# PeterFWS/Structure-PLP-SLAM

Hardware: AMD Instinct MI355X
Metric: frames/sec ORB+LSD extract+match, 640x480 TUM-RGBD, 1/2/4/8 GPU (higher is better)
Workload: dtype u8

## Files before the change

structure-plp-slam_amd/csrc/blur_tile.hpp:

```cpp
#pragma once
#include <hip/hip_runtime.h>
#include "plp_barrier.hpp"
#include <stdint.h>

namespace plp {

constexpr int kBlurTW = 128, kBlurTH = 32, kBlurPad = 8;
constexpr int kBlurRS = kBlurTH / 8;

__device__ __forceinline__ int blur_reflect101(int p, int len) {
    if (len == 1) return 0;
    p = p < 0 ? -p : p;
    p = p >= len ? 2 * (len - 1) - p : p;
    if (__builtin_expect(p < 0 || p >= len, 0))
        while (p < 0 || p >= len) p = p < 0 ? -p : 2 * (len - 1) - p;
    return p;
}

template <int R>
struct BlurTileLds {
    static constexpr int IW = kBlurTW + 2 * kBlurPad;
    static constexpr int IH = kBlurTH + 2 * R;
    static constexpr int NPR = IH / 2;
    uint8_t in[IH * IW];
    uint32_t hs2[NPR * kBlurTW];
};

typedef unsigned short blur_us2 __attribute__((ext_vector_type(2)));
__device__ __forceinline__ uint32_t blur_dot2(uint32_t a, uint32_t b, uint32_t c) {
    return __builtin_amdgcn_udot2(__builtin_bit_cast(blur_us2, a), __builtin_bit_cast(blur_us2, b), c, false);
}

template <int R, class Emit>
__device__ __forceinline__ void blur_tile_compute(BlurTileLds<R>& S, const int* __restrict__ taps, Emit emit) {
    constexpr int K = 2 * R + 1, IW = BlurTileLds<R>::IW, NPR = BlurTileLds<R>::NPR;
    const int tid = threadIdx.x;
    constexpr int RU = (R + 3) / 4 * 4;
    constexpr int OFF = RU - R;
    constexpr int ND = (OFF + 3 + K + 3) / 4;
    uint32_t tp[4][(K + 3 + 3) / 4];
#pragma unroll
    for (int e = 0; e < 4; ++e)
#pragma unroll
        for (int m = 0; m < (K + 3 + 3) / 4; ++m) {
            tp[e][m] = 0;
#pragma unroll
            for (int k = 0; k < 4; ++k) {
                const int t = 4 * m + k - e;
                if (t >= 0 && t < K) tp[e][m] |= (uint32_t)taps[t] << (8 * k);
            }
        }
    for (int i = tid; i < NPR * (kBlurTW / 4); i += 256) {
        const int p = i >> 5, c4 = (i & 31) * 4;
        uint32_t a[2][4];
#pragma unroll
        for (int rr = 0; rr < 2; ++rr) {
            const uint32_t* q = reinterpret_cast<const uint32_t*>(&S.in[(2 * p + rr) * IW + kBlurPad - RU + c4]);
            uint32_t d[ND];
#pragma unroll
            for (int k = 0; k < ND; ++k) d[k] = q[k];
#pragma unroll
            for (int o = 0; o < 4; ++o) {
                constexpr int dummy = 0; (void)dummy;
                const int s = OFF + o, q0 = s >> 2, e = s & 3;
                uint32_t acc = 0;
#pragma unroll
                for (int m = 0; m < (e + K + 3) / 4; ++m) acc = __builtin_amdgcn_udot4(d[q0 + m], tp[e][m], acc, false);
                a[rr][o] = acc;
            }
        }
        uint4 v;
        v.x = a[0][0] | (a[1][0] << 16); v.y = a[0][1] | (a[1][1] << 16); v.z = a[0][2] | (a[1][2] << 16); v.w = a[0][3] | (a[1][3] << 16);
        *reinterpret_cast<uint4*>(&S.hs2[p * kBlurTW + c4]) = v;
    }
    wg_barrier();
    const int cg = tid & 31, strip = tid >> 5;
    const int c4 = cg * 4, r0 = strip * kBlurRS;
    constexpr int NP = K / 2 + 1;
    uint32_t te[NP], to[NP];
#pragma unroll
    for (int j = 0; j < NP; ++j) {
        te[j] = (uint32_t)taps[2 * j] | (2 * j + 1 < K ? (uint32_t)taps[2 * j + 1] << 16 : 0u);
        to[j] = (j > 0 ? (uint32_t)taps[2 * j - 1] : 0u) | ((uint32_t)taps[2 * j] << 16);
    }
    uint4 wp[NP + 1];
#pragma unroll
    for (int j = 0; j <= NP; ++j) wp[j] = *reinterpret_cast<const uint4*>(&S.hs2[(r0 / 2 + j) * kBlurTW + c4]);
    uint32_t rows[kBlurRS];
#pragma unroll
    for (int rr = 0; rr < kBlurRS; ++rr) {
        uint32_t a0 = 32768u, a1 = 32768u, a2 = 32768u, a3 = 32768u;
#pragma unroll
        for (int j = 0; j < NP; ++j) {
            const uint32_t t = (rr & 1) ? to[j] : te[j];
            const uint4 v = wp[rr / 2 + j];
            a0 = blur_dot2(v.x, t, a0); a1 = blur_dot2(v.y, t, a1); a2 = blur_dot2(v.z, t, a2); a3 = blur_dot2(v.w, t, a3);
        }
        rows[rr] = __builtin_amdgcn_perm(a1, a0, 0x0c0c0602u) | __builtin_amdgcn_perm(a3, a2, 0x06020c0cu);
    }
    emit(r0, c4, rows);
}

struct BlurJob { const uint8_t* src; uint8_t* dst; int src_pitch, dst_pitch, w, h, tx0, ty0; };

template <int R> struct BlurPrefetch {
    static constexpr int IW = BlurTileLds<R>::IW, IH = BlurTileLds<R>::IH, DW = IW / 4;
    static constexpr int NPRE = (IH * DW + 255) / 256, NPATCH = (IH * 8 + 255) / 256;
    uint32_t pre[NPRE], patch[NPATCH];
};
template <int R> struct BlurSlot {
    static constexpr int DW = BlurTileLds<R>::IW / 4, QR = 256 / DW, QD = 256 % DW;
    static_assert((BlurPrefetch<R>::NPRE - 1) * QD + DW - 1 < 2 * DW, "a thread's dword index wraps at most once per step");
    int r0, d0;
    __device__ __forceinline__ BlurSlot() { const int tid = threadIdx.x; r0 = tid / DW; d0 = tid - r0 * DW; }
    __device__ __forceinline__ void at(int q, int& r, int& d) const { d = d0 + QD * q; r = r0 + QR * q; if (d >= DW) { d -= DW; ++r; } }
};
template <int R> __device__ __forceinline__ void blur_prefetch(BlurPrefetch<R>& F, const BlurJob& J) {
    constexpr int IW = BlurTileLds<R>::IW, IH = BlurTileLds<R>::IH, DW = IW / 4;
    const int tid = threadIdx.x;
    const BlurSlot<R> slot;
    const bool rows_inside = J.ty0 >= R && J.ty0 + kBlurTH + R <= J.h;
#pragma unroll
    for (int q = 0; q < BlurPrefetch<R>::NPRE; ++q) {
        int r, d;
        slot.at(q, r, d);
        const int x = J.tx0 - kBlurPad + 4 * d;
        int y = J.ty0 + r - R;
        if (!rows_inside) y = blur_reflect101(y, J.h);
        F.pre[q] = 0u;
        if (tid + 256 * q < IH * DW && x >= 0 && x + 3 < J.w) F.pre[q] = *reinterpret_cast<const uint32_t*>(J.src + (uint32_t)(__mul24(y, J.src_pitch) + x));
    }
    const int dr0 = (J.w - 3 - (J.tx0 - kBlurPad) + 3) >> 2;
    if (J.tx0 <= 0 || dr0 < DW) {
// ... 93 lines not shown
```

structure-plp-slam_amd/csrc/orb_context.hip:

```cpp
#include <hip/hip_runtime.h>

#include <algorithm>
#include <cstdio>
#include <cstring>
#include <mutex>
#include <string>
#include <vector>

#include "blur_tile.hpp"
#include "orb_device.hpp"
#include "xcd_map.hpp"
#include "plp_common.hpp"
#include "quadtree_model.hpp"

namespace plp {
void launch_quadtree(hipStream_t st, const LevelDev* d_lv, int n_levels, int n_cells_total, const uint32_t* cell_cand,
                     const int32_t* cell_count, int32_t* sel, int32_t* sel_count, int total_sel_cap, uint32_t* qt_scratch,
                     size_t qt_scratch_frame_stride, int32_t* status, int B, int max_quota);
size_t quadtree_scratch_bytes_per_frame(const LevelDev* h_lv, int n_levels);
}

using namespace plp;

struct plp_orb {
    HostPinned pin;
    plp_orb_params p{};
    std::vector<float> rects;
    int device = 0;
    hipStream_t stream = nullptr;
    OrbScaleTables st;
    OrbGeometry geo;
    std::vector<LevelDev> h_lv;
    int total_blur_tiles = 0;
    DevBuf d_lv, d_cells, d_rs;
    ResizeDev rs{};
    int capB = 0;
    DevBuf pyr, blur, l0copy, cell_cand, cell_count, sel, sel_count, status, qt_scratch, d_mask;
    size_t l0copy_frame_stride = 0, qt_frame_stride = 0;
    int max_quota = 0;
    DevBuf s_kps, s_desc, s_counts;
    DevBuf stereo_corr, stereo_stage;
    int s_cap = 0;
    bool mask_is_initialized = false;
    std::vector<uint8_t> rect_mask;
    int rect_mask_rows = 0, rect_mask_cols = 0;
    bool rect_mask_uploaded = false;
    DevBuf d_rect_mask;
    int last_B = 0;
    OrbPlanes last_planes{};
    hipStream_t last_stream = nullptr;
    bool profiling = false;
    hipEvent_t ev[8] = {};
    double stage_ms[7] = {0, 0, 0, 0, 0, 0, 0};
    long stage_batches = 0;
    std::mutex mu;
};

namespace {

plp_status validate(const plp_orb_params* p) {
    if (!p) return set_error(PLP_ERR_INVALID_ARG, "params is NULL");
    if (p->num_levels == 0 || p->num_levels > (uint32_t)kMaxLevels) return set_error(PLP_ERR_INVALID_ARG, "num_levels must be in [1,16]");
    if (!(p->scale_factor > 1.0f)) return set_error(PLP_ERR_INVALID_ARG, "scale_factor must be > 1");
    if (p->n_mask_rects < 0 || (p->n_mask_rects > 0 && !p->mask_rects)) return set_error(PLP_ERR_INVALID_ARG, "mask_rects");
    for (int i = 0; i < p->n_mask_rects; ++i) {
        const float* v = p->mask_rects + 4 * i;
        if (v[0] >= v[1]) return set_error(PLP_ERR_INVALID_ARG, "x_max must be greater than x_min");
        if (v[2] >= v[3]) return set_error(PLP_ERR_INVALID_ARG, "y_max must be greater than x_min");
    }
    return PLP_OK;
}

void reinitialize(plp_orb* c) {
    c->st = make_scale_tables(c->p.max_num_keypts, c->p.scale_factor, c->p.num_levels);
    c->geo = OrbGeometry{};
}

plp_status build_geometry_impl(plp_orb* c, int rows, int cols);

plp_status build_geometry(plp_orb* c, int rows, int cols) {
    if (c->geo.rows == rows && c->geo.cols == cols && c->geo.n_levels == (int)c->p.num_levels) return PLP_OK;
    const plp_status s = build_geometry_impl(c, rows, cols);
    if (s != PLP_OK) { c->geo = OrbGeometry{}; c->h_lv.clear(); c->capB = 0; }
    return s;
}

plp_status build_geometry_impl(plp_orb* c, int rows, int cols) {
    const int nl = (int)c->p.num_levels;
    {
        OrbGeometry g = make_geometry(rows, cols, c->st, nl);
        for (int l = 0; l < nl; ++l)
            if (g.lv[l].w <= 2 * kOrbBorder + 6 || g.lv[l].h <= 2 * kOrbBorder + 6)
                return set_error(PLP_ERR_INVALID_ARG, "image too small for the requested pyramid (level narrower than 45 px)");
        if (cols - 2 * kOrbBorder > 4095 || rows - 2 * kOrbBorder > 4095)
            return set_error(PLP_ERR_UNSUPPORTED, "images larger than 4133 px are not supported (12-bit candidate packing)");
        c->geo = std::move(g);
    }
    c->h_lv.assign(nl, LevelDev{});
    c->total_blur_tiles = 0;
    size_t qt_off = 0;
    int max_cells = 0;
    for (int l = 0; l < nl; ++l) {
        const LevelGeom& G = c->geo.lv[l];
        LevelDev& L = c->h_lv[l];
        L.w = G.w; L.h = G.h; L.pitch = G.pitch; L.off = G.off;
        L.blur_tiles = ((G.w + 127) / 128) * ((G.h + plp::kBlurTH - 1) / plp::kBlurTH);
        L.blur_tiles_x_magic = plp::plp_div_magic((uint32_t)((G.w + 127) / 128), (uint64_t)L.blur_tiles);
        c->total_blur_tiles += L.blur_tiles;
        L.scale = c->st.sf[l];
        L.sel_base = G.sel_base; L.sel_cap = G.sel_cap;
        L.cell_base = G.cell_base; L.n_cells = G.n_cell_rows * G.n_cell_cols;
        L.quota = (int)c->st.quota[l];
        c->max_quota = l == 0 ? L.quota : std::max(c->max_quota, L.quota);
        L.n_init_x = G.n_init_x; L.delta_x = G.delta_x; L.delta_y = G.delta_y;
        L.qt_cap = std::min(std::max(L.n_cells, 1) * kCellCap, 65535);
        L.qt_off = qt_off;
        qt_off += (size_t)L.qt_cap * 20;
        const int extent = (int)std::ceil(std::max(G.delta_x, G.delta_y)) + 1;
        int t1 = 0;
        while ((1 << t1) < extent) ++t1;
        const int d_eff = std::min(t1 + 2, kQtDepth);
        const int n_init = G.n_init_x * G.n_init_y;
        int nb = 0;
        while ((1 << nb) < n_init) ++nb;
        L.sort_lo = 2 * (kQtDepth - d_eff);
        L.sort_hi = 2 * kQtDepth + nb;
        if (L.n_cells > 2048 || 3 * L.quota + 8 > kQtMaxNodesLdsSmallBlock || n_init > 32)
            return set_error(PLP_ERR_UNSUPPORTED, "frame/keypoint budget exceeds the quadtree kernel limits (quota per level <= 2010, 2048 cells per level, 32 initial nodes)");
        max_cells = std::max(max_cells, L.n_cells);
    }
    if (3 * c->max_quota + 8 > kQtMaxNodesLds && max_cells > 1024)
        return set_error(PLP_ERR_UNSUPPORTED, "frame/keypoint budget exceeds the quadtree kernel limits (a quota above 1960 per level needs levels of at most 1024 cells)");
    PLP_HIP(c->d_lv.upload(c->h_lv.data(), sizeof(LevelDev) * nl, c->stream));
    PLP_HIP(c->d_cells.upload(c->geo.cells.data(), sizeof(CellDesc) * c->geo.cells.size(), c->stream));
    const ResizeTables& R = c->geo.rs;
    const size_t nc = R.xofs0.size(), nr = R.yofs0.size();
    std::vector<int16_t> blob;
    blob.reserve(4 * nc + 4 * nr + 8);
    auto push = [&](const std::vector<int16_t>& v) { size_t o = blob.size(); blob.insert(blob.end(), v.begin(), v.end()); return o; };
    const size_t o0 = push(R.xofs0), o1 = push(R.xofs1), o2 = push(R.a0), o3 = push(R.a1);
    const size_t o4 = push(R.yofs0), o5 = push(R.yofs1), o6 = push(R.b0), o7 = push(R.b1);
    if (blob.empty()) blob.push_back(0);
    PLP_HIP(c->d_rs.upload(blob.data(), blob.size() * 2, c->stream));
    const int16_t* base = (const int16_t*)c->d_rs.p;
    c->rs.xofs0 = base + o0; c->rs.xofs1 = base + o1; c->rs.a0 = base + o2; c->rs.a1 = base + o3;
    c->rs.yofs0 = base + o4; c->rs.yofs1 = base + o5; c->rs.b0 = base + o6; c->rs.b1 = base + o7;
    for (int l = 0; l < nl; ++l) { c->rs.col_base[l] = R.col_base[l]; c->rs.row_base[l] = R.row_base[l]; }
    c->capB = 0;
    PLP_HIP(hipStreamSynchronize(c->stream));
    return PLP_OK;
}

plp_status ensure_capacity(plp_orb* c, int B) {
    if (B <= c->capB) return PLP_OK;
    const OrbGeometry& g = c->geo;
    const size_t n_cells = g.cells.size();
    c->l0copy_frame_stride = ((size_t)g.lv[0].pitch * g.rows + 255) / 256 * 256;
    c->qt_frame_stride = quadtree_scratch_bytes_per_frame(c->h_lv.data(), g.n_levels);
    PLP_HIP(c->pyr.reserve(g.frame_plane_bytes * B));
    PLP_HIP(c->blur.reserve(g.frame_plane_bytes * B));
    PLP_HIP(c->l0copy.reserve(c->l0copy_frame_stride * B));
    PLP_HIP(c->cell_cand.reserve(sizeof(uint32_t) * kCellCap * n_cells * B));
    PLP_HIP(c->cell_count.reserve(sizeof(int32_t) * n_cells * B));
    PLP_HIP(c->sel.reserve(sizeof(int32_t) * g.total_sel_cap * B));
    PLP_HIP(c->sel_count.reserve(sizeof(int32_t) * kMaxLevels * B));
    PLP_HIP(c->status.reserve(sizeof(int32_t) * 4));
    PLP_HIP(c->qt_scratch.reserve(c->qt_frame_stride * B));
// ... 25 lines not shown

    const bool prof = c->profiling;
    static const bool trace = getenv("PLP_TRACE") != nullptr;
    auto mark = [&](int i) {
        if (prof) (void)hipEventRecord(c->ev[i], st);
        if (trace) { const hipError_t e = hipStreamSynchronize(st); fprintf(stderr, "plp_orb: stage boundary %d reached (%dx%d, B=%d)%s\n", i, cols, rows, B, e == hipSuccess ? "" : " ERROR"); fflush(stderr); }
    };
    mark(0);
    OrbPlanes pl{};
    pl.pyr = (uint8_t*)c->pyr.p; pl.pyr_frame_stride = g.frame_plane_bytes;
    const bool aligned = ((uintptr_t)d_imgs % 4 == 0) && (step % 4 == 0) && (frame_stride % 4 == 0);
    if (aligned) { pl.l0 = d_imgs; pl.l0_frame_stride = frame_stride; pl.l0_pitch = (int)step; }
    else {
        for (int f = 0; f < B; ++f)
            PLP_HIP(hipMemcpy2DAsync((uint8_t*)c->l0copy.p + f * c->l0copy_frame_stride, g.lv[0].pitch, d_imgs + f * frame_stride, step,
                                     cols, rows, hipMemcpyDeviceToDevice, st));
        pl.l0 = (const uint8_t*)c->l0copy.p; pl.l0_frame_stride = c->l0copy_frame_stride; pl.l0_pitch = g.lv[0].pitch;
    }
    build_rect_mask(c, rows, cols);
    if (!d_mask && !c->rect_mask.empty()) {
        if (c->rect_mask_rows != rows || c->rect_mask_cols != cols)
            return set_error(PLP_ERR_INVALID_ARG, "rectangle mask was built for a different frame size");
        if (!c->rect_mask_uploaded) {
            PLP_HIP(c->d_rect_mask.upload(c->rect_mask.data(), c->rect_mask.size(), st));
            c->rect_mask_uploaded = true;
        }
        d_mask = (const uint8_t*)c->d_rect_mask.p; mask_step = cols; mask_frame_stride = 0;
    }

    PLP_HIP(hipMemsetAsync(c->status.p, 0, 16, st));
    mark(1);
    for (int l = 1; l < nl; ++l) launch_resize(st, pl, c->h_lv.data(), l, B, c->rs);
    mark(2);
    launch_fast(st, pl, (const CellDesc*)c->d_cells.p, (int)g.cells.size(), (const LevelDev*)c->d_lv.p, B, (int)c->p.ini_fast_thr,
                (int)c->p.min_fast_thr, d_mask, mask_step, mask_frame_stride, (uint32_t*)c->cell_cand.p, (int32_t*)c->cell_count.p);
    mark(3);
    BlurTaps taps{{18, 34, 48, 56, 48, 34, 18}};
    launch_blur(st, pl, (uint8_t*)c->blur.p, g.frame_plane_bytes, (const LevelDev*)c->d_lv.p, nl, c->total_blur_tiles, B, taps, c->h_lv.data());
    mark(4);
    launch_quadtree(st, (const LevelDev*)c->d_lv.p, nl, (int)g.cells.size(), (const uint32_t*)c->cell_cand.p,
                    (const int32_t*)c->cell_count.p, (int32_t*)c->sel.p, (int32_t*)c->sel_count.p, g.total_sel_cap,
                    (uint32_t*)c->qt_scratch.p, c->qt_frame_stride, (int32_t*)c->status.p, B, c->max_quota);
    mark(5);
    UMax um;
    for (int v = 0; v <= kHalfPatch; ++v) um.v[v] = c->st.u_max[v];
    launch_orient_rbrief(st, pl, (const uint8_t*)c->blur.p, g.frame_plane_bytes, (const LevelDev*)c->d_lv.p, nl, (const int32_t*)c->sel.p,
                         (const int32_t*)c->sel_count.p, g.total_sel_cap, um, d_kps, d_desc, cap, d_counts, (int32_t*)c->status.p, B);
    PLP_HIP(hipGetLastError());
    if (trace) { const hipError_t e = hipStreamSynchronize(st); fprintf(stderr, "plp_orb: batch done%s\n", e == hipSuccess ? "" : " ERROR"); fflush(stderr); }
    if (prof) {
        mark(6);
        PLP_HIP(hipEventSynchronize(c->ev[6]));
        for (int i = 0; i < 6; ++i) { float ms = 0; PLP_HIP(hipEventElapsedTime(&ms, c->ev[i], c->ev[i + 1])); c->stage_ms[i] += ms; }
        float tot = 0; PLP_HIP(hipEventElapsedTime(&tot, c->ev[0], c->ev[6])); c->stage_ms[6] += tot;
        ++c->stage_batches;
    }
    c->last_B = B; c->last_planes = pl; c->last_stream = st;
    return PLP_OK;
}

}

extern "C" {

void plp_orb_default_params(plp_orb_params* p) {
    if (!p) return;
    p->max_num_keypts = 2000; p->scale_factor = 1.2f; p->num_levels = 8; p->ini_fast_thr = 20; p->min_fast_thr = 7;
    p->mask_rects = nullptr; p->n_mask_rects = 0;
}

plp_status plp_orb_create(const plp_orb_params* params, int device, plp_orb** out) {
// ... 294 lines not shown
```

structure-plp-slam_amd/csrc/orb_device.hpp:

```cpp
#pragma once
#include <hip/hip_runtime.h>
#include <stdint.h>

#include "../../include/plp_front.h"
#include "orb_tables.hpp"

namespace plp {

constexpr int kQtMaxNodesLds = 5888;
constexpr int kQtMaxNodesLdsSmallBlock = 6040;

struct LevelDev {
    int w, h, pitch;
    int blur_tiles;
    uint32_t blur_tiles_x_magic;
    size_t off;
    float scale;
    int sel_base, sel_cap;
    int cell_base, n_cells;
    int quota;
    int n_init_x;
    double delta_x, delta_y;
    size_t qt_off;
    int qt_cap;
    int sort_lo, sort_hi;
};

struct OrbPlanes {
    const uint8_t* l0; size_t l0_frame_stride; int l0_pitch;
    uint8_t* pyr; size_t pyr_frame_stride;
    __host__ __device__ const uint8_t* level_ptr(int frame, int level, const LevelDev& L) const {
        return level == 0 ? l0 + (size_t)frame * l0_frame_stride : pyr + (size_t)frame * pyr_frame_stride + L.off;
    }
    __host__ __device__ int level_pitch(int level, const LevelDev& L) const { return level == 0 ? l0_pitch : L.pitch; }
};

struct BlurTaps { int k[7]; };
struct UMax { int v[kHalfPatch + 1]; };

struct ResizeDev {
    const int16_t *xofs0, *xofs1, *a0, *a1, *yofs0, *yofs1, *b0, *b1;
    int col_base[kMaxLevels], row_base[kMaxLevels];
};

struct StereoArgs {
    const plp_keypoint *kps_l, *kps_r;
    const uint8_t *desc_l, *desc_r;
    const int32_t *cnt_l, *cnt_r;
    int cap;
    float fxb, tb;
    float inv_scale[kMaxLevels];
    float* x_right; float* depth;
    int32_t* corr;
};
void launch_stereo(hipStream_t st, const OrbPlanes& pl_l, const OrbPlanes& pl_r, const LevelDev* d_lv, const StereoArgs& A, int B);

void launch_resize(hipStream_t st, const OrbPlanes& pl, const LevelDev* h_lv, int level, int B, const ResizeDev& rs);
void launch_fast(hipStream_t st, const OrbPlanes& pl, const CellDesc* d_cells, int n_cells, const LevelDev* d_lv, int B,
                 int ini_thr, int min_thr, const uint8_t* d_mask, size_t mask_step, size_t mask_frame_stride,
                 uint32_t* cell_cand, int32_t* cell_count);
void launch_blur(hipStream_t st, const OrbPlanes& pl, uint8_t* blur, size_t blur_frame_stride, const LevelDev* d_lv,
                 int n_levels, int total_tiles, int B, const BlurTaps& taps, const LevelDev* h_lv = nullptr);
void launch_orient_rbrief(hipStream_t st, const OrbPlanes& pl, const uint8_t* blur, size_t blur_frame_stride,
                          const LevelDev* d_lv, int n_levels, const int32_t* sel, const int32_t* sel_count,
                          int total_sel_cap, const UMax& um, plp_keypoint* kps, uint8_t* desc, int cap, int32_t* counts,
                          int32_t* status, int B);

}
```

structure-plp-slam_amd/csrc/orb_kernels.hip:

```cpp
#include <hip/hip_runtime.h>
#include <stdint.h>

#include "blur_tile.hpp"
#include "plp_barrier.hpp"
#include "orb_device.hpp"
#include "plp_common.hpp"
#include "xcd_map.hpp"

namespace plp {

__device__ __forceinline__ int rs_tab(const int16_t* __restrict__ t, int i) { return *reinterpret_cast<const int16_t*>(reinterpret_cast<const char*>(t) + ((uint32_t)i << 1)); }
constexpr int kRsRows = 44, kRsPitch = 96;

__global__ __launch_bounds__(256) __attribute__((amdgpu_waves_per_eu(7, 8))) void k_resize_linear(const uint8_t* __restrict__ src_base, size_t src_frame_stride,
                                                       int src_pitch, int sw, uint8_t* __restrict__ dst_base,
                                                       size_t dst_frame_stride, int dst_pitch, int dw, int dh,
                                                       const int16_t* __restrict__ xofs0, const int16_t* __restrict__ xofs1,
                                                       const int16_t* __restrict__ a0, const int16_t* __restrict__ a1,
                                                       const int16_t* __restrict__ yofs0, const int16_t* __restrict__ yofs1,
                                                       const int16_t* __restrict__ b0, const int16_t* __restrict__ b1) {
    constexpr int ROWS = 8;
    __shared__ __attribute__((aligned(16))) uint8_t tiles[4 * kRsRows * kRsPitch];
    const int lane = threadIdx.x & 63, wv = __builtin_amdgcn_readfirstlane((int)(threadIdx.x >> 6));
    const int strip_x0 = blockIdx.x * 64, strip_y0 = (blockIdx.y * 4 + wv) * 32;
// ... 78 lines not shown
            cached_row = y1;
            *reinterpret_cast<uint32_t*>(dst + (uint32_t)(__mul24(dy, dst_pitch) + dx0)) = packed;
        }
        return;
    }
    for (int r = 0; r < ROWS; ++r) {
        const int dy = dy0 + r;
        if (dy >= dh) break;
        const uint8_t* S0 = src + (size_t)yofs0[dy] * src_pitch;
        const uint8_t* S1 = src + (size_t)yofs1[dy] * src_pitch;
        const int wb0 = b0[dy], wb1 = b1[dy];
        uint32_t packed = 0;
#pragma unroll
        for (int i = 0; i < 4; ++i) {
            const int h0 = S0[x0[i]] * wa0[i] + S0[x1[i]] * wa1[i];
            const int h1 = S1[x0[i]] * wa0[i] + S1[x1[i]] * wa1[i];
            const int v = (((wb0 * (h0 >> 4)) >> 16) + ((wb1 * (h1 >> 4)) >> 16) + 2) >> 2;
            packed |= (uint32_t)(v & 255) << (8 * i);
        }
        *reinterpret_cast<uint32_t*>(dst + (size_t)dy * dst_pitch + dx0) = packed;
    }
}

constexpr int kFastQ1 = 1536, kFastQ2 = 512;
constexpr int kTileW = 76;
constexpr int kScoreW = 68;

__device__ __forceinline__ int min3(int a, int b, int c) { return min(a, min(b, c)); }

__global__ __launch_bounds__(256) __attribute__((amdgpu_waves_per_eu(8, 8))) void k_fast_cells(OrbPlanes pl, const CellDesc* __restrict__ cells,
                                                    const LevelDev* __restrict__ lv, int ini_thr, int min_thr,
                                                    const uint8_t* __restrict__ mask, size_t mask_step,
                                                    size_t mask_frame_stride, uint32_t* __restrict__ cell_cand,
                                                    int32_t* __restrict__ cell_count, int n_cells, uint32_t gx_magic) {
    __shared__ __attribute__((aligned(16))) uint8_t tile[70 * kTileW];
    __shared__ __attribute__((aligned(16))) uint8_t score[66 * kScoreW];
    __shared__ unsigned long long keepbits[64];
    __shared__ uint16_t queue[kFastQ1], queue2[kFastQ2];
    __shared__ unsigned long long bits1[64], bits2[64];
    __shared__ int q_count, q2_count, n_ini, wave_tot[4], run_base;

    unsigned ucell, uframe;
    xcd_frame_major(ucell, uframe, gx_magic);
    const int tid = threadIdx.x, frame = (int)uframe, cell = (int)ucell;
    const CellDesc cd = cells[cell];
    const LevelDev L = lv[cd.level];
    const int out_slot = frame * n_cells + cell;
    const float sf = L.scale;

    const uint8_t* mk = mask ? mask + (size_t)frame * mask_frame_stride : nullptr;
    auto masked = [&](int y, int x) -> bool {
        return mk[(size_t)(int)((float)y * sf) * mask_step + (int)((float)x * sf)] == 0;
    };
    if (mk) {
        const int x0 = cd.min_x, x1 = cd.min_x + cd.w, y0 = cd.min_y, y1 = cd.min_y + cd.h;
        if (masked(y0, x0) || masked(y1, x0) || masked(y0, x1) || masked(y1, x1)) {
            if (tid == 0) cell_count[out_slot] = 0;
            return;
        }
    }

    const uint8_t* img = pl.level_ptr(frame, cd.level, L);
    const int pitch = pl.level_pitch(cd.level, L);
    const int w = cd.w, h = cd.h;
    {
        const int a0 = cd.min_x - 1;
        const int sh = a0 & 3;
        const int ndw = (w + 2 + 3) >> 2;
        const uint8_t* row0 = img + (size_t)cd.min_y * pitch + (a0 - sh);
        const int qr = 256 / ndw, qd = 256 - qr * ndw;
        int r = tid / ndw, c = tid - r * ndw;
        for (int i = tid; i < ndw * h; i += 256, c += qd, r += qr) {
            if (c >= ndw) { c -= ndw; ++r; }
            const uint32_t* g = reinterpret_cast<const uint32_t*>(row0 + (ptrdiff_t)(__mul24(r, pitch) + 4 * c));
            const uint32_t lo = g[0];
            const uint32_t v = sh ? __builtin_amdgcn_alignbyte(g[1], lo, (uint32_t)sh) : lo;
            *reinterpret_cast<uint32_t*>(&tile[r * kTileW + 4 * c]) = v;
        }
    }
    const int tw = w - 6, th = h - 6;
    int thr = ini_thr;
    for (int attempt = 0; attempt < 2; ++attempt) {
        thr = attempt == 0 ? ini_thr : min_thr;
        for (int i = tid; i < 66 * kScoreW / 4; i += 256) reinterpret_cast<uint32_t*>(score)[i] = 0;
        if (tid < 64) { keepbits[tid] = 0ull; bits1[tid] = 0ull; bits2[tid] = 0ull; }
        if (tid == 0) { q_count = 0; q2_count = 0; n_ini = 0; run_base = 0; }
        wg_barrier();
        for (int i = tid; i < 1024; i += 256) {
            const int ty = i >> 4, tx4 = (i & 15) * 4;
            if (tx4 >= tw || ty >= th) continue;
            const uint32_t* rowc = reinterpret_cast<const uint32_t*>(&tile[(ty + 3) * kTileW]) + (tx4 >> 2);
            const uint32_t C = rowc[1], Lw = rowc[0], Rw = rowc[2];
            const uint32_t Lq = __builtin_amdgcn_alignbyte(C, Lw, 1u);
            const uint32_t Rq = __builtin_amdgcn_alignbyte(Rw, C, 3u);
            const uint32_t U = *(reinterpret_cast<const uint32_t*>(&tile[ty * kTileW]) + (tx4 >> 2) + 1);
            const uint32_t D = *(reinterpret_cast<const uint32_t*>(&tile[(ty + 6) * kTileW]) + (tx4 >> 2) + 1);
#pragma unroll
            for (int k = 0; k < 4; ++k) {
                if (tx4 + k >= tw) break;
                const int v = (int)((C >> (8 * k)) & 255u);
                const int hi = v + thr, lo = v - thr;
                const int p0 = (int)((D >> (8 * k)) & 255u), p4 = (int)((Rq >> (8 * k)) & 255u), p8 = (int)((U >> (8 * k)) & 255u),
                          p12 = (int)((Lq >> (8 * k)) & 255u);
                const bool b0 = p0 > hi, b4 = p4 > hi, b8 = p8 > hi, b12 = p12 > hi;
                const bool d0 = p0 < lo, d4 = p4 < lo, d8 = p8 < lo, d12 = p12 < lo;
                if (((b0 | b8) & (b4 | b12)) | ((d0 | d8) & (d4 | d12))) {
                    atomicOr(&bits1[ty], 1ull << (tx4 + k));
                    const int slot = atomicAdd(&q_count, 1);
                    if (slot < kFastQ1) queue[slot] = (uint16_t)((ty << 6) | (tx4 + k));
                }
            }
        }
        wg_barrier();
// ... 117 lines not shown
    wg_barrier();
    int off = 0;
    for (int k = 0; k < wv; ++k) off += wave_tot[k];
    for (int ty = 16 * wv; ty < 16 * wv + 16; ++ty) {
        const unsigned long long m = row_mask(ty);
        if ((m >> lane) & 1ull) {
            const uint32_t v = score[(ty + 1) * kScoreW + lane + 1];
            const uint32_t x = (uint32_t)(lane + 3 + cd.cx * kCellSize), y = (uint32_t)(ty + 3 + cd.cy * kCellSize);
            out[off + __popcll(m & ((1ull << lane) - 1ull))] = x | (y << 12) | (v << 24);
        }
        off += __popcll(m);
    }
    if (tid == 0) run_base = wave_tot[0] + wave_tot[1] + wave_tot[2] + wave_tot[3];
    wg_barrier();
    if (tid == 0) cell_count[out_slot] = run_base;
}

__global__ __launch_bounds__(256) __attribute__((amdgpu_waves_per_eu(8, 8))) void k_blur7(OrbPlanes pl, uint8_t* __restrict__ blur_base, size_t blur_frame_stride,
                                               const LevelDev* __restrict__ lv, int n_levels, BlurTaps taps, uint32_t gx_magic) {
    __shared__ BlurTileLds<3> S;
    unsigned ut, uf;
    xcd_frame_major(ut, uf, gx_magic);
    int t = (int)ut;
    const int frame = (int)uf;
    int level = 0;
    while (level + 1 < n_levels && t >= lv[level].blur_tiles) { t -= lv[level].blur_tiles; ++level; }
    const LevelDev L = lv[level];
    const int tiles_x = (L.w + kBlurTW - 1) / kBlurTW;
    const int trow = (int)plp_div((unsigned)t, (unsigned)tiles_x, L.blur_tiles_x_magic);
    blur_tile<3>(S, pl.level_ptr(frame, level, L), pl.level_pitch(level, L), blur_base + (size_t)frame * blur_frame_stride + L.off, L.pitch,
                 L.w, L.h, (t - trow * tiles_x) * kBlurTW, trow * kBlurTH, taps.k);
}

__device__ __forceinline__ float fast_atan2_deg(float y, float x) {
    const float p1 = 0.9997878412794807f * (float)(180 / 3.14159265358979323846);
    const float p3 = -0.3258083974640975f * (float)(180 / 3.14159265358979323846);
    const float p5 = 0.1555786518463281f * (float)(180 / 3.14159265358979323846);
    const float p7 = -0.04432655554792128f * (float)(180 / 3.14159265358979323846);
    const float eps = (float)2.2204460492503131e-16;
    const float ax = fabsf(x), ay = fabsf(y);
    float a;
    if (ax >= ay) {
        const float c = __fdiv_rn(ay, __fadd_rn(ax, eps));
        const float c2 = __fmul_rn(c, c);
        a = __fmul_rn(__fadd_rn(__fmul_rn(__fadd_rn(__fmul_rn(__fadd_rn(__fmul_rn(p7, c2), p5), c2), p3), c2), p1), c);
    } else {
        const float c = __fdiv_rn(ax, __fadd_rn(ay, eps));
        const float c2 = __fmul_rn(c, c);
        a = __fsub_rn(90.f, __fmul_rn(__fadd_rn(__fmul_rn(__fadd_rn(__fmul_rn(__fadd_rn(__fmul_rn(p7, c2), p5), c2), p3), c2), p1), c));
    }
    if (x < 0) a = __fsub_rn(180.f, a);
    if (y < 0) a = __fsub_rn(360.f, a);
    return a;
}

__device__ __forceinline__ float ref_poly_cos(float v) {
    const float v2 = __fmul_rn(v, v);
    return __fadd_rn(0.99940307f, __fmul_rn(v2, __fadd_rn(-0.49558072f, __fmul_rn(0.03679168f, v2))));
}
__device__ __forceinline__ float ref_cos(float v) {
    const float PI = 3.14159265358979f, PI_2 = PI / 2.0f, TWO_PI = 2.0f * PI, INV_TWO_PI = 1.0f / TWO_PI, THREE_PI_2 = 3.0f * PI_2;
    const float q = __fmul_rn(v, INV_TWO_PI);
    int fl = (int)q;
    fl -= (fl > q);
    v = __fsub_rn(v, __fmul_rn((float)fl, TWO_PI));
    v = (0.0f < v) ? v : -v;
// ... 137 lines not shown
    }
#pragma unroll
    for (int r = 0; r < 16; ++r) bits |= (uint32_t)(ta[r] < tb[r]) << r;
    reinterpret_cast<uint16_t*>(out_desc + ((size_t)frame * cap + out_idx) * 32)[sub] = (uint16_t)bits;
    if (sub == 0) {
        plp_keypoint k;
        const float s = L.scale;
        k.x = level ? __fmul_rn((float)cx, s) : (float)cx;
        k.y = level ? __fmul_rn((float)cy, s) : (float)cy;
        k.size = (float)(unsigned)(__fmul_rn((float)kFastPatch, s));
        k.angle = angle;
        k.response = (float)resp;
        k.octave = level;
        k.class_id = -1;
        out_kps[(size_t)frame * cap + out_idx] = k;
    }
}

void launch_resize(hipStream_t st, const OrbPlanes& pl, const LevelDev* h_lv, int level, int B, const ResizeDev& rs) {
    const LevelDev& S = h_lv[level - 1];
    const LevelDev& D = h_lv[level];
    const uint8_t* src = level - 1 == 0 ? pl.l0 : pl.pyr + S.off;
    const size_t sstride = level - 1 == 0 ? pl.l0_frame_stride : pl.pyr_frame_stride;
    const int spitch = level - 1 == 0 ? pl.l0_pitch : S.pitch;
    dim3 grid((D.w + 63) / 64, (D.h + 127) / 128, B), block(256);
    hipLaunchKernelGGL(k_resize_linear, grid, block, 0, st, src, sstride, spitch, S.w, pl.pyr + D.off, pl.pyr_frame_stride, D.pitch,
                       D.w, D.h, rs.xofs0 + rs.col_base[level], rs.xofs1 + rs.col_base[level], rs.a0 + rs.col_base[level],
                       rs.a1 + rs.col_base[level], rs.yofs0 + rs.row_base[level], rs.yofs1 + rs.row_base[level],
                       rs.b0 + rs.row_base[level], rs.b1 + rs.row_base[level]);
}

void launch_fast(hipStream_t st, const OrbPlanes& pl, const CellDesc* d_cells, int n_cells, const LevelDev* d_lv, int B,
                 int ini_thr, int min_thr, const uint8_t* d_mask, size_t mask_step, size_t mask_frame_stride,
                 uint32_t* cell_cand, int32_t* cell_count) {
    hipLaunchKernelGGL(k_fast_cells, dim3(n_cells, B), dim3(256), 0, st, pl, d_cells, d_lv, ini_thr, min_thr, d_mask, mask_step,
                       mask_frame_stride, cell_cand, cell_count, n_cells, plp_div_magic((uint32_t)n_cells, (uint64_t)n_cells * B));
}

void launch_blur(hipStream_t st, const OrbPlanes& pl, uint8_t* blur, size_t blur_frame_stride, const LevelDev* d_lv,
                 int n_levels, int total_tiles, int B, const BlurTaps& taps, const LevelDev* h_lv) {
    (void)h_lv;
    hipLaunchKernelGGL(k_blur7, dim3(total_tiles, B), dim3(256), 0, st, pl, blur, blur_frame_stride, d_lv, n_levels, taps, plp_div_magic((uint32_t)total_tiles, (uint64_t)total_tiles * B));
}

void launch_orient_rbrief(hipStream_t st, const OrbPlanes& pl, const uint8_t* blur, size_t blur_frame_stride,
                          const LevelDev* d_lv, int n_levels, const int32_t* sel, const int32_t* sel_count,
                          int total_sel_cap, const UMax& um, plp_keypoint* kps, uint8_t* desc, int cap, int32_t* counts,
                          int32_t* status, int B) {
    hipLaunchKernelGGL(k_orient_rbrief, dim3((total_sel_cap + 15) / 16, B), dim3(256), 0, st, pl, blur, blur_frame_stride, d_lv,
                       n_levels, sel, sel_count, total_sel_cap, um, kps, desc, cap, counts, status,
                       plp_div_magic((uint32_t)((total_sel_cap + 15) / 16), (uint64_t)((total_sel_cap + 15) / 16) * B));
}

__global__ __launch_bounds__(256) void k_stereo_match(OrbPlanes pl_l, OrbPlanes pl_r, const LevelDev* __restrict__ lv, StereoArgs A) {
    const int lane = threadIdx.x & 63, b = blockIdx.y;
    const int il = blockIdx.x * 4 + __builtin_amdgcn_readfirstlane((int)(threadIdx.x >> 6));
    const int nl = A.cnt_l ? min(A.cnt_l[b], A.cap) : A.cap, nr = A.cnt_r ? min(A.cnt_r[b], A.cap) : A.cap;
    if (il >= A.cap) return;
    float* xr_out = A.x_right + (size_t)b * A.cap;
    float* dp_out = A.depth + (size_t)b * A.cap;
    int32_t* corr_out = A.corr + (size_t)b * A.cap;
    if (lane == 0) { xr_out[il] = -1.0f; dp_out[il] = -1.0f; corr_out[il] = -1; }
    if (il >= nl) return;
    const plp_keypoint kp = A.kps_l[(size_t)b * A.cap + il];
    const plp_keypoint* kr = A.kps_r + (size_t)b * A.cap;
    const float max_disp = __fdiv_rn(A.fxb, A.tb), min_disp = 0.0f;
    const int row = (int)(unsigned long long)kp.y;
    const float min_x = __fsub_rn(kp.x, max_disp), max_x = __fsub_rn(kp.x, min_disp);
    if (max_x < 0) return;
// ... 106 lines not shown
```

structure-plp-slam_amd/csrc/orb_tables.hpp:

```cpp
#pragma once
#include <algorithm>
#include <cmath>
#include <cstdint>
#include <vector>

namespace plp {

constexpr int kOrbBorder = 19;
constexpr int kFastPatch = 31;
constexpr int kHalfPatch = 15;
constexpr int kCellSize = 64;
constexpr int kCellOverlap = 6;
constexpr int kMaxLevels = 16;
constexpr int kCellCap = 1024;

struct OrbScaleTables {
    std::vector<float> sf, isf, sigma2, isigma2;
    std::vector<uint32_t> quota;
    int u_max[kHalfPatch + 1];
};

inline OrbScaleTables make_scale_tables(uint32_t max_kp, float scale_factor, uint32_t n_levels) {
    OrbScaleTables t;
    t.sf.assign(n_levels, 1.0f); t.isf.assign(n_levels, 1.0f);
// ... 18 lines not shown
    t.quota[n_levels - 1] = (uint32_t)std::max((int)max_kp - (int)used, 0);
    const double r = kHalfPatch;
    const int vmax = (int)std::floor(r * std::sqrt(2.0) / 2 + 1);
    const int vmin = (int)std::ceil(r * std::sqrt(2.0) / 2);
    for (int v = 0; v <= kHalfPatch; ++v) t.u_max[v] = 0;
    for (int v = 0; v <= vmax; ++v) t.u_max[v] = (int)std::round(std::sqrt(r * r - (double)v * v));
    for (int v = kHalfPatch, v0 = 0; v >= vmin; --v) {
        while (t.u_max[v0] == t.u_max[v0 + 1]) ++v0;
        t.u_max[v] = v0;
        ++v0;
    }
    return t;
}

inline int floor_i(float v) { int i = (int)v; return i - (i > v); }
inline short q11(float w) {
    const int i = (int)std::nearbyintf(w * 2048);
    return (short)std::min(std::max(i, -32768), 32767);
}

struct LevelGeom {
    int w = 0, h = 0, pitch = 0;
    size_t off = 0;
    int n_cell_cols = 0, n_cell_rows = 0;
    int cell_base = 0;
    int max_bx = 0, max_by = 0;
    int n_init_x = 1, n_init_y = 1;
    double delta_x = 0, delta_y = 0;
    int sel_cap = 0, sel_base = 0;
};

struct CellDesc {
    int32_t level, min_x, min_y, w;
    int32_t h, cx, cy, pad;
};

struct ResizeTables {
    std::vector<int16_t> xofs0, xofs1, a0, a1;
    std::vector<int16_t> yofs0, yofs1, b0, b1;
    std::vector<int> col_base, row_base;
};

struct OrbGeometry {
    int rows = 0, cols = 0, n_levels = 0;
    std::vector<LevelGeom> lv;
    std::vector<CellDesc> cells;
    size_t frame_plane_bytes = 0;
    int total_sel_cap = 0;
    ResizeTables rs;
};

inline OrbGeometry make_geometry(int rows, int cols, const OrbScaleTables& st, int n_levels) {
    OrbGeometry g;
    g.rows = rows; g.cols = cols; g.n_levels = n_levels;
    g.lv.resize(n_levels);
    size_t off = 0;
    for (int l = 0; l < n_levels; ++l) {
        LevelGeom& L = g.lv[l];
        if (l == 0) { L.w = cols; L.h = rows; }
        else {
            const double scale = st.sf[l];
            L.w = (int)std::round(cols * 1.0 / scale);
            L.h = (int)std::round(rows * 1.0 / scale);
        }
        L.pitch = (L.w + 63) / 64 * 64;
        L.off = off;
        off += ((size_t)L.pitch * L.h + 255) / 256 * 256;
// ... 76 lines not shown
```

Before: 91500.

## Fuse Gaussian blur into FAST cell kernel, blur only uncovered borders separately

The FAST cell kernel already loads each cell's image tile into LDS, so it now also computes the 7-tap Gaussian blur of the cell interior from that tile and writes it out. This avoids a second read of the pyramid by the separate blur pass. A new border kernel blurs only the strips not covered by cell interiors, using wide or tall tiles. The old full blur path stays available through an environment variable. The cost is more LDS pressure and extra work and barriers in the FAST kernel, and the border kernel adds a launch.

```diff
diff --git a/structure-plp-slam_amd/csrc/blur_tile.hpp b/structure-plp-slam_amd/csrc/blur_tile.hpp
--- a/structure-plp-slam_amd/csrc/blur_tile.hpp
+++ b/structure-plp-slam_amd/csrc/blur_tile.hpp
@@ -31,9 +31,10 @@
     return __builtin_amdgcn_udot2(__builtin_bit_cast(blur_us2, a), __builtin_bit_cast(blur_us2, b), c, false);
 }
 
-template <int R, class Emit>
-__device__ __forceinline__ void blur_tile_compute(BlurTileLds<R>& S, const int* __restrict__ taps, Emit emit) {
-    constexpr int K = 2 * R + 1, IW = BlurTileLds<R>::IW, NPR = BlurTileLds<R>::NPR;
+template <int R, int TW, int IP, class Emit>
+__device__ __forceinline__ void blur_block_compute(const uint8_t* in0, uint32_t* hs2, const int* __restrict__ taps, Emit emit) {
+    constexpr int K = 2 * R + 1, CG = TW / 4, TH = 4096 / TW, NPR = TH / 2 + R;
+    static_assert((CG & (CG - 1)) == 0 && CG <= 256 && IP % 4 == 0, "column groups: a power of two");
     const int tid = threadIdx.x;
     constexpr int RU = (R + 3) / 4 * 4;
     constexpr int OFF = RU - R;
@@ -50,12 +51,12 @@
                 if (t >= 0 && t < K) tp[e][m] |= (uint32_t)taps[t] << (8 * k);
             }
         }
-    for (int i = tid; i < NPR * (kBlurTW / 4); i += 256) {
-        const int p = i >> 5, c4 = (i & 31) * 4;
+    for (int i = tid; i < NPR * CG; i += 256) {
+        const int p = (int)((unsigned)i / CG), c4 = (int)((unsigned)i % CG) * 4;
         uint32_t a[2][4];
 #pragma unroll
         for (int rr = 0; rr < 2; ++rr) {
-            const uint32_t* q = reinterpret_cast<const uint32_t*>(&S.in[(2 * p + rr) * IW + kBlurPad - RU + c4]);
+            const uint32_t* q = reinterpret_cast<const uint32_t*>(&in0[(2 * p + rr) * IP + c4]);
             uint32_t d[ND];
 #pragma unroll
             for (int k = 0; k < ND; ++k) d[k] = q[k];
@@ -71,10 +72,10 @@
         }
         uint4 v;
         v.x = a[0][0] | (a[1][0] << 16); v.y = a[0][1] | (a[1][1] << 16); v.z = a[0][2] | (a[1][2] << 16); v.w = a[0][3] | (a[1][3] << 16);
-        *reinterpret_cast<uint4*>(&S.hs2[p * kBlurTW + c4]) = v;
+        *reinterpret_cast<uint4*>(&hs2[p * TW + c4]) = v;
     }
     wg_barrier();
-    const int cg = tid & 31, strip = tid >> 5;
+    const int cg = (int)((unsigned)tid % CG), strip = (int)((unsigned)tid / CG);
     const int c4 = cg * 4, r0 = strip * kBlurRS;
     constexpr int NP = K / 2 + 1;
     uint32_t te[NP], to[NP];
@@ -85,7 +86,7 @@
     }
     uint4 wp[NP + 1];
 #pragma unroll
-    for (int j = 0; j <= NP; ++j) wp[j] = *reinterpret_cast<const uint4*>(&S.hs2[(r0 / 2 + j) * kBlurTW + c4]);
+    for (int j = 0; j <= NP; ++j) wp[j] = *reinterpret_cast<const uint4*>(&hs2[(r0 / 2 + j) * TW + c4]);
     uint32_t rows[kBlurRS];
 #pragma unroll
     for (int rr = 0; rr < kBlurRS; ++rr) {
@@ -99,6 +100,13 @@
         rows[rr] = __builtin_amdgcn_perm(a1, a0, 0x0c0c0602u) | __builtin_amdgcn_perm(a3, a2, 0x06020c0cu);
     }
     emit(r0, c4, rows);
+}
+
+template <int R, class Emit>
+__device__ __forceinline__ void blur_tile_compute(BlurTileLds<R>& S, const int* __restrict__ taps, Emit emit) {
+    constexpr int RU = (R + 3) / 4 * 4;
+    static_assert(4096 / kBlurTW == kBlurTH && BlurTileLds<R>::NPR == kBlurTH / 2 + R, "tile shape");
+    blur_block_compute<R, kBlurTW, BlurTileLds<R>::IW>(&S.in[kBlurPad - RU], S.hs2, taps, emit);
 }
 
 struct BlurJob { const uint8_t* src; uint8_t* dst; int src_pitch, dst_pitch, w, h, tx0, ty0; };
diff --git a/structure-plp-slam_amd/csrc/orb_context.hip b/structure-plp-slam_amd/csrc/orb_context.hip
--- a/structure-plp-slam_amd/csrc/orb_context.hip
+++ b/structure-plp-slam_amd/csrc/orb_context.hip
@@ -32,7 +32,8 @@
     OrbGeometry geo;
     std::vector<LevelDev> h_lv;
     int total_blur_tiles = 0;
-    DevBuf d_lv, d_cells, d_rs;
+    std::vector<BlurStrip> blur_strips;
+    DevBuf d_lv, d_cells, d_rs, d_strips;
     ResizeDev rs{};
     int capB = 0;
     DevBuf pyr, blur, l0copy, cell_cand, cell_count, sel, sel_count, status, qt_scratch, d_mask;
@@ -77,6 +78,40 @@
 }
 
 plp_status build_geometry_impl(plp_orb* c, int rows, int cols);
+
+void build_blur_coverage(std::vector<CellDesc>& cells, const std::vector<LevelDev>& lv, std::vector<BlurStrip>& strips) {
+    strips.clear();
+    auto add = [&](int l, int x0, int x1, int y0, int y1, bool wide) {
+        if (x0 >= x1 || y0 >= y1) return;
+        const int tw = wide ? kBlurTW : 4096 / kBlurTW, th = 4096 / tw;
+        for (int ty = y0; ty < y1; ty += th)
+            for (int tx = x0 & ~3; tx < x1; tx += tw) strips.push_back({l, tx, ty, wide ? 1 : 0, x0, x1, y0, y1});
+    };
+    for (int l = 0; l < (int)lv.size(); ++l) {
+        const LevelDev& L = lv[l];
+        int ix0 = L.w, ix1 = 0, iy0 = L.h, iy1 = 0;
+        long long area = 0;
+        for (int k = L.cell_base; k < L.cell_base + L.n_cells; ++k) {
+            const CellDesc& a = cells[k];
+            ix0 = std::min(ix0, a.min_x + 3); ix1 = std::max(ix1, a.min_x + a.w - 3);
+            iy0 = std::min(iy0, a.min_y + 3); iy1 = std::max(iy1, a.min_y + a.h - 3);
+            area += (long long)(a.w - 6) * (a.h - 6);
+        }
+        bool tiled = L.n_cells > 0 && ix0 >= 3 && iy0 >= 3 && ix1 <= L.w - 3 && iy1 <= L.h - 3 && area == (long long)(ix1 - ix0) * (iy1 - iy0);
+        for (int k = L.cell_base; tiled && k < L.cell_base + L.n_cells; ++k)
+            for (int m = k + 1; tiled && m < L.cell_base + L.n_cells; ++m) {
+                const CellDesc &a = cells[k], &b = cells[m];
+                tiled = a.w <= 6 || b.w <= 6 || a.h <= 6 || b.h <= 6 || a.min_x + a.w - 3 <= b.min_x + 3 || b.min_x + b.w - 3 <= a.min_x + 3 ||
+                        a.min_y + a.h - 3 <= b.min_y + 3 || b.min_y + b.h - 3 <= a.min_y + 3;
+            }
+        for (int k = L.cell_base; k < L.cell_base + L.n_cells; ++k) cells[k].blur = tiled ? 1 : 0;
+        if (!tiled) { add(l, 0, L.w, 0, L.h, true); continue; }
+        add(l, 0, L.w, 0, iy0, true);
+        add(l, 0, L.w, iy1, L.h, true);
+        add(l, 0, ix0, iy0, iy1, false);
+        add(l, ix1, L.w, iy0, iy1, false);
+    }
+}
 
 plp_status build_geometry(plp_orb* c, int rows, int cols) {
     if (c->geo.rows == rows && c->geo.cols == cols && c->geo.n_levels == (int)c->p.num_levels) return PLP_OK;
@@ -131,8 +166,10 @@
     }
     if (3 * c->max_quota + 8 > kQtMaxNodesLds && max_cells > 1024)
         return set_error(PLP_ERR_UNSUPPORTED, "frame/keypoint budget exceeds the quadtree kernel limits (a quota above 1960 per level needs levels of at most 1024 cells)");
+    build_blur_coverage(c->geo.cells, c->h_lv, c->blur_strips);
     PLP_HIP(c->d_lv.upload(c->h_lv.data(), sizeof(LevelDev) * nl, c->stream));
     PLP_HIP(c->d_cells.upload(c->geo.cells.data(), sizeof(CellDesc) * c->geo.cells.size(), c->stream));
+    if (!c->blur_strips.empty()) PLP_HIP(c->d_strips.upload(c->blur_strips.data(), sizeof(BlurStrip) * c->blur_strips.size(), c->stream));
     const ResizeTables& R = c->geo.rs;
     const size_t nc = R.xofs0.size(), nr = R.yofs0.size();
     std::vector<int16_t> blob;
@@ -224,11 +261,17 @@
     mark(1);
     for (int l = 1; l < nl; ++l) launch_resize(st, pl, c->h_lv.data(), l, B, c->rs);
     mark(2);
+    static const bool separate_blur = [] { const char* e = getenv("PLP_ORB_BLUR"); return e && strcmp(e, "separate") == 0; }();
+    const BlurTaps taps{{18, 34, 48, 56, 48, 34, 18}};
     launch_fast(st, pl, (const CellDesc*)c->d_cells.p, (int)g.cells.size(), (const LevelDev*)c->d_lv.p, B, (int)c->p.ini_fast_thr,
-                (int)c->p.min_fast_thr, d_mask, mask_step, mask_frame_stride, (uint32_t*)c->cell_cand.p, (int32_t*)c->cell_count.p);
+                (int)c->p.min_fast_thr, d_mask, mask_step, mask_frame_stride, (uint32_t*)c->cell_cand.p, (int32_t*)c->cell_count.p,
+                separate_blur ? nullptr : (uint8_t*)c->blur.p, g.frame_plane_bytes, taps);
     mark(3);
-    BlurTaps taps{{18, 34, 48, 56, 48, 34, 18}};
-    launch_blur(st, pl, (uint8_t*)c->blur.p, g.frame_plane_bytes, (const LevelDev*)c->d_lv.p, nl, c->total_blur_tiles, B, taps, c->h_lv.data());
+    if (separate_blur)
+        launch_blur(st, pl, (uint8_t*)c->blur.p, g.frame_plane_bytes, (const LevelDev*)c->d_lv.p, nl, c->total_blur_tiles, B, taps, c->h_lv.data());
+    else
+        launch_blur_border(st, pl, (uint8_t*)c->blur.p, g.frame_plane_bytes, (const LevelDev*)c->d_lv.p, (const BlurStrip*)c->d_strips.p,
+                           (int)c->blur_strips.size(), B, taps);
     mark(4);
     launch_quadtree(st, (const LevelDev*)c->d_lv.p, nl, (int)g.cells.size(), (const uint32_t*)c->cell_cand.p,
                     (const int32_t*)c->cell_count.p, (int32_t*)c->sel.p, (int32_t*)c->sel_count.p, g.total_sel_cap,
diff --git a/structure-plp-slam_amd/csrc/orb_device.hpp b/structure-plp-slam_amd/csrc/orb_device.hpp
--- a/structure-plp-slam_amd/csrc/orb_device.hpp
+++ b/structure-plp-slam_amd/csrc/orb_device.hpp
@@ -36,6 +36,8 @@
 };
 
 struct BlurTaps { int k[7]; };
+
+struct BlurStrip { int level, tx0, ty0, wide, x0, x1, y0, y1; };
 struct UMax { int v[kHalfPatch + 1]; };
 
 struct ResizeDev {
@@ -58,7 +60,9 @@
 void launch_resize(hipStream_t st, const OrbPlanes& pl, const LevelDev* h_lv, int level, int B, const ResizeDev& rs);
 void launch_fast(hipStream_t st, const OrbPlanes& pl, const CellDesc* d_cells, int n_cells, const LevelDev* d_lv, int B,
                  int ini_thr, int min_thr, const uint8_t* d_mask, size_t mask_step, size_t mask_frame_stride,
-                 uint32_t* cell_cand, int32_t* cell_count);
+                 uint32_t* cell_cand, int32_t* cell_count, uint8_t* blur, size_t blur_frame_stride, const BlurTaps& taps);
+void launch_blur_border(hipStream_t st, const OrbPlanes& pl, uint8_t* blur, size_t blur_frame_stride, const LevelDev* d_lv,
+                        const BlurStrip* d_strips, int n_strips, int B, const BlurTaps& taps);
 void launch_blur(hipStream_t st, const OrbPlanes& pl, uint8_t* blur, size_t blur_frame_stride, const LevelDev* d_lv,
                  int n_levels, int total_tiles, int B, const BlurTaps& taps, const LevelDev* h_lv = nullptr);
 void launch_orient_rbrief(hipStream_t st, const OrbPlanes& pl, const uint8_t* blur, size_t blur_frame_stride,
diff --git a/structure-plp-slam_amd/csrc/orb_kernels.hip b/structure-plp-slam_amd/csrc/orb_kernels.hip
--- a/structure-plp-slam_amd/csrc/orb_kernels.hip
+++ b/structure-plp-slam_amd/csrc/orb_kernels.hip
@@ -134,12 +134,21 @@
                                                     const LevelDev* __restrict__ lv, int ini_thr, int min_thr,
                                                     const uint8_t* __restrict__ mask, size_t mask_step,
                                                     size_t mask_frame_stride, uint32_t* __restrict__ cell_cand,
-                                                    int32_t* __restrict__ cell_count, int n_cells, uint32_t gx_magic) {
+                                                    int32_t* __restrict__ cell_count, int n_cells, uint32_t gx_magic,
+                                                    uint8_t* __restrict__ blur_base, size_t blur_frame_stride, BlurTaps taps) {
     __shared__ __attribute__((aligned(16))) uint8_t tile[70 * kTileW];
-    __shared__ __attribute__((aligned(16))) uint8_t score[66 * kScoreW];
+    struct FastScratch {
+        uint8_t score[66 * kScoreW];
+        uint16_t queue[kFastQ1], queue2[kFastQ2];
+        unsigned long long bits1[64], bits2[64];
+    };
+    __shared__ __attribute__((aligned(16))) union { FastScratch f; uint32_t hs2[(32 + 3) * 64]; } U;
+    auto& score = U.f.score;
     __shared__ unsigned long long keepbits[64];
-    __shared__ uint16_t queue[kFastQ1], queue2[kFastQ2];
-    __shared__ unsigned long long bits1[64], bits2[64];
+    auto& queue = U.f.queue;
+    auto& queue2 = U.f.queue2;
+    auto& bits1 = U.f.bits1;
+    auto& bits2 = U.f.bits2;
     __shared__ int q_count, q2_count, n_ini, wave_tot[4], run_base;
 
     unsigned ucell, uframe;
@@ -154,11 +163,14 @@
     auto masked = [&](int y, int x) -> bool {
         return mk[(size_t)(int)((float)y * sf) * mask_step + (int)((float)x * sf)] == 0;
     };
+    const bool blur_cell = blur_base != nullptr && cd.blur != 0;
+    bool skipped = false;
     if (mk) {
         const int x0 = cd.min_x, x1 = cd.min_x + cd.w, y0 = cd.min_y, y1 = cd.min_y + cd.h;
         if (masked(y0, x0) || masked(y1, x0) || masked(y0, x1) || masked(y1, x1)) {
             if (tid == 0) cell_count[out_slot] = 0;
-            return;
+            if (!blur_cell) return;
+            skipped = true;
         }
     }
 
@@ -181,6 +193,27 @@
         }
     }
     const int tw = w - 6, th = h - 6;
+    if (blur_cell) {
+        static_assert((kOrbBorder + 3) % 2 == 0 && kCellSize % 4 == 0, "interior columns start 2-byte aligned: 16-bit stores");
+        wg_barrier();
+        uint8_t* dst = blur_base + (size_t)frame * blur_frame_stride + L.off + (size_t)(cd.min_y + 3) * L.pitch + (cd.min_x + 3);
+        blur_block_compute<3, 64, kTileW>(tile, U.hs2, taps.k, [&](int r0, int c4, const uint32_t (&rows)[kBlurRS]) {
+            const int n = min(tw - c4, 4);
+            if (n <= 0) return;
+#pragma unroll
+            for (int rr = 0; rr < kBlurRS; ++rr) {
+                if (r0 + rr >= th) break;
+                uint8_t* p = dst + (uint32_t)__mul24(r0 + rr, L.pitch) + c4;
+                if (n == 4) {
+                    reinterpret_cast<uint16_t*>(p)[0] = (uint16_t)rows[rr];
+                    reinterpret_cast<uint16_t*>(p)[1] = (uint16_t)(rows[rr] >> 16);
+                } else
+                    for (int k = 0; k < n; ++k) p[k] = (uint8_t)(rows[rr] >> (8 * k));
+            }
+        });
+        wg_barrier();
+        if (skipped) return;
+    }
     int thr = ini_thr;
     for (int attempt = 0; attempt < 2; ++attempt) {
         thr = attempt == 0 ? ini_thr : min_thr;
@@ -364,6 +397,78 @@
                  L.w, L.h, (t - trow * tiles_x) * kBlurTW, trow * kBlurTH, taps.k);
 }
 
+struct BorderEmit {
+    uint8_t* dst; int pitch, tx0, ty0, x0, x1, y0, y1;
+    __device__ __forceinline__ void operator()(int r0, int c4, const uint32_t (&rows)[kBlurRS]) const {
+        const int x = tx0 + c4;
+        if (x >= x1 || x + 4 <= x0) return;
+        const bool whole = x >= x0 && x + 4 <= x1;
+#pragma unroll
+        for (int rr = 0; rr < kBlurRS; ++rr) {
+            const int y = ty0 + r0 + rr;
+            if (y < y0 || y >= y1) continue;
+            uint8_t* p = dst + (size_t)y * pitch + x;
+            if (whole) *reinterpret_cast<uint32_t*>(p) = rows[rr];
+            else
+                for (int k = 0; k < 4; ++k)
+                    if (x + k >= x0 && x + k < x1) p[k] = (uint8_t)(rows[rr] >> (8 * k));
+        }
+    }
+};
+
+struct TallLds {
+    static constexpr int TW = 32, TH = 4096 / TW, IW = TW + 8, IH = TH + 6;
+    uint8_t in[IH * IW];
+    __attribute__((aligned(16))) uint32_t hs2[(TH / 2 + 3) * TW];
+};
+
+__device__ __forceinline__ void blur7_tall_tile(TallLds& S, const uint8_t* __restrict__ src, int src_pitch, int w, int h, int tx0, int ty0,
+                                                const int* __restrict__ taps, const BorderEmit& emit) {
+    constexpr int IW = TallLds::IW, IH = TallLds::IH, DW = IW / 4, N = IH * DW, NQ = (N + 255) / 256;
+    const int tid = threadIdx.x;
+    uint32_t v[NQ];
+    const uint8_t* rowp[NQ];
+#pragma unroll
+    for (int q = 0; q < NQ; ++q) {
+        const int i = min(tid + 256 * q, N - 1), r = (int)((unsigned)i / DW), d = i - r * DW;
+        rowp[q] = src + (size_t)blur_reflect101(ty0 - 3 + r, h) * src_pitch;
+        v[q] = *reinterpret_cast<const uint32_t*>(rowp[q] + min(max(tx0 - 4 + 4 * d, 0), w - 4));
+    }
+#pragma unroll
+    for (int q = 0; q < NQ; ++q) {
+        const int i = min(tid + 256 * q, N - 1), r = (int)((unsigned)i / DW), d = i - r * DW;
+        const int x = tx0 - 4 + 4 * d;
+        if (x < 0 || x + 3 >= w) {
+            uint32_t b = 0u;
+#pragma unroll
+            for (int k = 0; k < 4; ++k) b |= (uint32_t)rowp[q][blur_reflect101(x + k, w)] << (8 * k);
+            v[q] = b;
+        }
+    }
+#pragma unroll
+    for (int q = 0; q < NQ; ++q) {
+        const int i = tid + 256 * q, r = (int)((unsigned)i / DW), d = i - r * DW;
+        if (i < N) *reinterpret_cast<uint32_t*>(&S.in[r * IW + 4 * d]) = v[q];
+    }
+    wg_barrier();
+    blur_block_compute<3, TallLds::TW, IW>(S.in, S.hs2, taps, emit);
+}
+
+__global__ __launch_bounds__(256) __attribute__((amdgpu_waves_per_eu(8, 8))) void k_blur7_border(OrbPlanes pl, uint8_t* __restrict__ blur_base, size_t blur_frame_stride,
+                                                      const LevelDev* __restrict__ lv, const BlurStrip* __restrict__ strips, BlurTaps taps, uint32_t gx_magic) {
+    __shared__ __attribute__((aligned(16))) union { BlurTileLds<3> wide; TallLds tall; } S;
+    unsigned ut, uf;
+    xcd_frame_major(ut, uf, gx_magic);
+    const int frame = (int)uf;
+    const BlurStrip J = strips[ut];
+    const LevelDev L = lv[J.level];
+    const uint8_t* src = pl.level_ptr(frame, J.level, L);
+    const int src_pitch = pl.level_pitch(J.level, L);
+    const BorderEmit emit{blur_base + (size_t)frame * blur_frame_stride + L.off, L.pitch, J.tx0, J.ty0, J.x0, J.x1, J.y0, J.y1};
+    if (J.wide) blur_tile_core<3>(S.wide, src, src_pitch, L.w, L.h, J.tx0, J.ty0, taps.k, emit);
+    else blur7_tall_tile(S.tall, src, src_pitch, L.w, L.h, J.tx0, J.ty0, taps.k, emit);
+}
+
 __device__ __forceinline__ float fast_atan2_deg(float y, float x) {
     const float p1 = 0.9997878412794807f * (float)(180 / 3.14159265358979323846);
     const float p3 = -0.3258083974640975f * (float)(180 / 3.14159265358979323846);
@@ -567,9 +672,17 @@
 
 void launch_fast(hipStream_t st, const OrbPlanes& pl, const CellDesc* d_cells, int n_cells, const LevelDev* d_lv, int B,
                  int ini_thr, int min_thr, const uint8_t* d_mask, size_t mask_step, size_t mask_frame_stride,
-                 uint32_t* cell_cand, int32_t* cell_count) {
+                 uint32_t* cell_cand, int32_t* cell_count, uint8_t* blur, size_t blur_frame_stride, const BlurTaps& taps) {
     hipLaunchKernelGGL(k_fast_cells, dim3(n_cells, B), dim3(256), 0, st, pl, d_cells, d_lv, ini_thr, min_thr, d_mask, mask_step,
-                       mask_frame_stride, cell_cand, cell_count, n_cells, plp_div_magic((uint32_t)n_cells, (uint64_t)n_cells * B));
+                       mask_frame_stride, cell_cand, cell_count, n_cells, plp_div_magic((uint32_t)n_cells, (uint64_t)n_cells * B),
+                       blur, blur_frame_stride, taps);
+}
+
+void launch_blur_border(hipStream_t st, const OrbPlanes& pl, uint8_t* blur, size_t blur_frame_stride, const LevelDev* d_lv,
+                        const BlurStrip* d_strips, int n_strips, int B, const BlurTaps& taps) {
+    if (n_strips <= 0) return;
+    hipLaunchKernelGGL(k_blur7_border, dim3(n_strips, B), dim3(256), 0, st, pl, blur, blur_frame_stride, d_lv, d_strips, taps,
+                       plp_div_magic((uint32_t)n_strips, (uint64_t)n_strips * B));
 }
 
 void launch_blur(hipStream_t st, const OrbPlanes& pl, uint8_t* blur, size_t blur_frame_stride, const LevelDev* d_lv,
diff --git a/structure-plp-slam_amd/csrc/orb_tables.hpp b/structure-plp-slam_amd/csrc/orb_tables.hpp
--- a/structure-plp-slam_amd/csrc/orb_tables.hpp
+++ b/structure-plp-slam_amd/csrc/orb_tables.hpp
@@ -74,7 +74,8 @@
 
 struct CellDesc {
     int32_t level, min_x, min_y, w;
-    int32_t h, cx, cy, pad;
+    int32_t h, cx, cy;
+    int32_t blur;
 };
 
 struct ResizeTables {
```

Result: faster. 92660, median of 6 (+1.3%).
